# ZhengyiLuo/UHC

Measured on NVIDIA H100. Metric: env_steps_per_s, higher is better.
Workload: dtype f32

## Files before the change

### __graft_entry__.py

```python
import os
import subprocess
import sys

ROOT = os.path.dirname(os.path.abspath(__file__))
if ROOT not in sys.path:
    sys.path.insert(0, ROOT)


def build():
    from uhc_b200 import build as b
    b.build()
    from oracle import oracle as O
    O.build()
    from tests.emu import curriculum_emu, emu, eval_emu, export_emu, group_emu, motion_emu, render_emu, render_mesh_emu, subject_emu, track_emu, video_emu
    emu.build()
    motion_emu.build()
    export_emu.build()
    eval_emu.build()
    curriculum_emu.build()
    track_emu.build()
    group_emu.build()
    render_emu.build()
    render_mesh_emu.build()
    video_emu.build()
    subject_emu.build()
    import uhc_b200
    from uhc_b200 import model
    model.HumanoidModel()


# ... 47 lines not shown
```

### uhc_b200/csrc/env_step.h

```cpp
#pragma once
#include "sim_core.h"
#include "curriculum_core.h"

namespace uhc {

struct CurView {
    const float *pct;
    const int *start;
    const int *meta;
    int max_freq, fit_clip;
    float prec_freq;
};

template <class Real>
struct EngineView {
    Model<Real> model;
    EnvCfg<Real> cfg;
    int num_envs;
    Real *state;
    int *istate;
    const Real *expert;
    const int *clip_adr;
    const Real *clip_shape;
    const int *clip_model;
    const float *clip_cdf;
    const Real *neutral;
    int *ep_log;
    int *ep_start_log;
    int *counters;
    CurView cur;
#if defined(UHC_PHASE_CLOCKS) && !defined(UHC_EMU)
    long long *phase_cyc;
#endif
};

template <class Real>
UHC_DEV bool env_record_valid(const EngineView<Real> &ev, int env) {
    const int *is = ev.istate + (size_t)env * SI_SIZE;
    const int clip = is[SI_CLIP], len = is[SI_LEN];
    return len >= 2 && clip >= 0 && clip < ev.cfg.num_clips;
}
template <class Real, class ObsT>
UHC_DEV void env_step_invalid(const EngineView<Real> &ev, ObsT *obs, ObsT *reward, ObsT *cinfo_out, int *fail_out, int *end_out, ObsT *percent_out) {
    LANES_BEGIN
    if (obs) for (int i = lane; i < ev.cfg.obs_dim; i += 32) obs[i] = (ObsT)0;
    if (cinfo_out && lane < 5) cinfo_out[lane] = (ObsT)0;
    if (lane == 0) {
// ... 273 lines not shown
    LANES_END
    store_state(ev, env, w);
    if (ev.cfg.auto_reset && (fail || end)) {
        int nclip, nstart, nlen;
        const int episode = is[SI_EPISODE] + 1;
        if constexpr (CUR) sample_clip_cur(ev, env, episode, &nclip, &nstart, &nlen);
        else sample_clip(ev, env, episode, &nclip, &nstart, &nlen);
        env_reset_warp<Real, ObsT>(ev, env, w, nclip, nstart, nlen, (const Real *)nullptr, (const Real *)nullptr, obs);
        LANES_BEGIN
        if (lane == 0) is[SI_EPISODE] = episode;
        LANES_END
    }
#if defined(UHC_PHASE_CLOCKS) && !defined(UHC_EMU)
    PCLK(true, w, PC_EPILOGUE);
    if (ev.phase_cyc && (threadIdx.x & 31) == 0) for (int i = 0; i < NPHASE; i++) ev.phase_cyc[(size_t)env * NPHASE + i] += w.pc[i];
#endif
    return fail || end;
}

}
```

### uhc_b200/csrc/sim_core.h

```cpp
#pragma once
#include <math.h>
#include <stdint.h>

#ifndef UHC_EMU
#include <cuda_runtime.h>
#define UHC_DEV __device__ __forceinline__
#define UHC_DEVNI __device__ __noinline__
#define LANES_BEGIN { const int lane = (int)(threadIdx.x & 31);
#define LANES_END } __syncwarp();
#define LANES_END_R }
#define LVAR(T, n) T n
#define LV(n) n
#define LVARA(T, n, K) T n[K]
#define LVA(n) n
#define LV_ARR(n, c) n[c]
#define LV_ALL(n) n
#define UHC_LDG(p) __ldg(p)
__device__ __forceinline__ float uhc_lds(const float *p) { float v; asm("ld.shared.f32 %0, [%1];" : "=f"(v) : "r"((unsigned)__cvta_generic_to_shared(p))); return v; }
__device__ __forceinline__ double uhc_lds(const double *p) { double v; asm("ld.shared.f64 %0, [%1];" : "=d"(v) : "r"((unsigned)__cvta_generic_to_shared(p))); return v; }
__device__ __forceinline__ int uhc_lds(const int *p) { int v; asm("ld.shared.s32 %0, [%1];" : "=r"(v) : "r"((unsigned)__cvta_generic_to_shared(p))); return v; }
#define UHC_LDT(p) uhc_lds(p)
#else
#define UHC_DEV static inline
#define UHC_DEVNI static
// ... 50 lines not shown
    int auto_reset, t_min, t_max, num_clips;
    unsigned long long reset_seed;
    int reactive_v; Real reactive_rate;
    int rfc_mode, vf_dim, act_dim;
    int obs_v, obs_dim;
    int fut_frames, fut_skip;
    int has_shape, obs_block;
    signed char vf_slot[NB];
    int term_body, head_body;
    int reward_mul;
};
constexpr int VF_BODY_DIM = 9, MAX_ACT_DIM = NU + VF_BODY_DIM * NB + 30;

enum { PC_LOAD, PC_PD, PC_KIN, PC_COLLIDE, PC_SMOOTH, PC_CSETUP, PC_NEWTON_ABA, PC_NEWTON_ROWS, PC_SYNC_SUBSTEP, PC_SYNC_PD, PC_SYNC_SMOOTH,
       PC_INTEGRATE, PC_EPILOGUE, NPHASE };

template <class Real>
struct Work {
    alignas(16) Real q[NQ]; Real v[NV + 1], aw[NV + 1], C[NV + 1];
    Real Ib[NB][10];
    alignas(16) Real S[NV + 6][6];
    alignas(16) Real xpos[NB][3]; Real xipos[NB][3], xmat[NB][9];
    Real act[ACT_DIM + 3];
    union {
        struct {
            alignas(16) Real aU[NV + 6][6];
            Real au[NV + 6];
        };
        struct {
            alignas(16) Real xquat[NB][4];
// ... 3 lines not shown
    };
    Real as_[NV + 1], a[NV + 1], g[NV + 1], p[NV + 1], Mp[NV + 1], tau[NV + 1];
    alignas(16) Real Ab[NB][6];
    int cbody[MAXCON]; Real cr[MAXCON][3], cdist[MAXCON], cD[MAXCON], caref[MAXCON][4], cres[MAXCON][4], cjp[MAXCON][4];
    int bcon_adr[NB + 1];
    int ncon, upper_contact;
    int nlim;
    int con_overflow;
    alignas(8) unsigned long long mbar;
    int sync_threads;
    int sync_id;
    alignas(8) Model<Real> mdl;
    alignas(8) EnvCfg<Real> cfg;
#if defined(UHC_PHASE_CLOCKS) && !defined(UHC_EMU)
    long long pc_t, pc[NPHASE];
#endif
};

#if defined(UHC_PHASE_CLOCKS) && !defined(UHC_EMU)
#define PCLK_START(w) do { __syncwarp(); if ((threadIdx.x & 31) == 0) { for (int i_ = 0; i_ < NPHASE; i_++) (w).pc[i_] = 0; (w).pc_t = clock64(); } } while (0)
#define PCLK(on, w, ph) do { if (on) { __syncwarp(); if ((threadIdx.x & 31) == 0) { const long long t_ = clock64(); (w).pc[ph] += t_ - (w).pc_t; (w).pc_t = t_; } } } while (0)
#else
#define PCLK_START(w) do { } while (0)
#define PCLK(on, w, ph) do { (void)sizeof(on); } while (0)
#endif

UHC_DEV float rcp_(float x) {
#if defined(__CUDA_ARCH__)
    float r; asm("rcp.approx.ftz.f32 %0, %1;" : "=f"(r) : "f"(x)); return fmaf(r, fmaf(-x, r, 1.0f), r);
#else
    return 1.0f / x;
#endif
}
UHC_DEV double rcp_(double x) { return 1.0 / x; }
UHC_DEV float rsqrt_(float x) { return 1.0f / sqrtf(x); }
UHC_DEV double rsqrt_(double x) { return 1.0 / sqrt(x); }
UHC_DEV void sincos_(float x, float *s, float *c) {
    const float k = rintf(x * 0.63661977236758134f);
    float r = fmaf(k, -1.5707962512969971f, x);
// ... 93 lines not shown
template <class R> UHC_DEV R warp_sum(R x) {
#pragma unroll 1
    for (int o = 16; o; o >>= 1) x += __shfl_xor_sync(0xffffffffu, x, o);
    return x;
}
template <class R> UHC_DEV R warp_max(R x) { for (int o = 16; o; o >>= 1) { R y = __shfl_xor_sync(0xffffffffu, x, o); x = x > y ? x : y; } return x; }
template <class R> UHC_DEV void warp_argmin(R &x, int &i) {
    for (int o = 16; o; o >>= 1) { R y = __shfl_xor_sync(0xffffffffu, x, o); int j = __shfl_xor_sync(0xffffffffu, i, o); if (y < x || (y == x && j < i)) { x = y; i = j; } }
}
#define WSUM(n) warp_sum(n)
#define WMAX(n) warp_max(n)
#define WARGMIN(x, i, ox, oi) { ox = x; oi = i; warp_argmin(ox, oi); }
#define WBALLOT(n) __ballot_sync(0xffffffffu, (n) != 0)
UHC_DEV int warp_excl_scan(int x, int lane) { int p = x; for (int o = 1; o < 32; o <<= 1) { const int t = __shfl_up_sync(0xffffffffu, p, o); if (lane >= o) p += t; } return p - x; }
#define WEXSCAN(dst, src) { dst = warp_excl_scan(src, (int)(threadIdx.x & 31)); }
template <class R, int K> UHC_DEV void subtree_sum(R (&x)[K], int sub_end, int lane) {
#pragma unroll 1
    for (int o = 1; o < 32; o <<= 1) {
#pragma unroll
        for (int i = 0; i < K; i++) { const R t = __shfl_up_sync(0xffffffffu, x[i], o); if (lane >= o) x[i] += t; }
    }
#pragma unroll
    for (int i = 0; i < K; i++) {
        const R hi = __shfl_sync(0xffffffffu, x[i], sub_end), lo = __shfl_up_sync(0xffffffffu, x[i], 1);
        x[i] = hi - (lane > 0 ? lo : R(0));
    }
}
template <class R, int K> UHC_DEV void ancestor_sum(R (&x)[K], int a1, int a2, int a4, int a8) {
    static_assert(MAXLEVEL + 1 <= 16, "four pointer-jumping rounds cover chains of 16 bodies");
#pragma unroll 1
// ... 10 lines not shown
#pragma unroll
        for (int i = 0; i < K; i++) { const R t = __shfl_up_sync(0xffffffffu, x[i], o); if (lane >= o) x[i] += t; }
    }
}
#define WPREFIX(n, K) prefix_sum<Real, K>(n, (int)(threadIdx.x & 31))
#define WANCESTOR(n, K, tp) ancestor_sum<Real, K>(n, tp.parent, tp.anc2, tp.anc4, tp.anc8)
#else
template <class R> static R emu_sum(const R *x) { R s = 0; for (int i = 0; i < 32; i++) s += x[i]; return s; }
template <class R> static R emu_max(const R *x) { R s = x[0]; for (int i = 1; i < 32; i++) s = x[i] > s ? x[i] : s; return s; }
#define WSUM(n) emu_sum(n)
#define WMAX(n) emu_max(n)
#define WARGMIN(x, i, ox, oi) { ox = x[0]; oi = i[0]; for (int l_ = 1; l_ < 32; l_++) if (x[l_] < ox || (x[l_] == ox && i[l_] < oi)) { ox = x[l_]; oi = i[l_]; } }
static unsigned emu_ballot(const int *x) { unsigned m = 0; for (int i = 0; i < 32; i++) if (x[i]) m |= 1u << i; return m; }
#define WBALLOT(n) emu_ballot(n)
#define WEXSCAN(dst, src) { int run_ = 0; for (int l_ = 0; l_ < 32; l_++) { const int t_ = src[l_]; dst[l_] = run_; run_ += t_; } }
template <class R, int K, class TP> static void emu_subtree(R (*x)[K], const TP *tp) {
    R out[32][K];
    for (int b = 0; b < 32; b++) for (int i = 0; i < K; i++) { R s = 0; for (int c = b; c <= tp[b].sub_end && c < 32; c++) s += x[c][i]; out[b][i] = s; }
    for (int b = 0; b < 32; b++) for (int i = 0; i < K; i++) x[b][i] = out[b][i];
}
template <class R, int K, class TP> static void emu_ancestor(R (*x)[K], const TP *tp) {
    for (int b = 1; b < NB; b++) for (int i = 0; i < K; i++) x[b][i] += x[tp[b].parent][i];
}
#define WSUBTREE(n, K, tp) emu_subtree<Real, K>(n, tp)
#define WPREFIX(n, K) { for (int l_ = 1; l_ < 32; l_++) for (int i_ = 0; i_ < K; i_++) n[l_][i_] += n[l_ - 1][i_]; }
#define WANCESTOR(n, K, tp) emu_ancestor<Real, K>(n, tp)
#endif
UHC_DEV int popc_(unsigned x) { int c = 0; while (x) { x &= x - 1; c++; } return c; }

struct LaneTopo { signed char lane, parent, depth, sub_end, ch0, ch1, ch2, anc2, anc4, anc8; short hnum; int hadr; };
template <class Real>
UHC_DEV LaneTopo lane_topo(const Model<Real> &m, int lane) {
    LaneTopo t; t.lane = lane;
    const int b = lane < NB ? lane : NB - 1;
    t.parent = UHC_LDG(m.parent + b); t.depth = lane < NB ? UHC_LDG(m.depth + b) : 99; t.sub_end = lane < NB ? UHC_LDG(m.body_sub_end + b) : lane;
    const int c0 = UHC_LDG(m.child_adr + b), c1 = UHC_LDG(m.child_adr + b + 1);
    t.ch0 = (lane < NB && c0 < c1) ? UHC_LDG(m.child + c0) : -1;
    t.ch1 = (lane < NB && c0 + 1 < c1) ? UHC_LDG(m.child + c0 + 1) : -1;
    t.ch2 = (lane < NB && c0 + 2 < c1) ? UHC_LDG(m.child + c0 + 2) : -1;
    t.hadr = UHC_LDG(m.hull_adr + b); t.hnum = lane < NB ? UHC_LDG(m.hull_num + b) : 0;
    int a = lane < NB ? b : -1;
    t.anc2 = t.anc4 = t.anc8 = -1;
    for (int k = 1; k <= 8 && a >= 0; ++k) { a = a > 0 ? UHC_LDG(m.parent + a) : -1; if (k == 2) t.anc2 = a; if (k == 4) t.anc4 = a; if (k == 8) t.anc8 = a; }
// ... 243 lines not shown
            paxpy6(x0, S0, a); paxpy6(x1, S1, a); paxpy6(x2, S2, a);
            if (b == 0 && r == 0) {
                x[0] = a[1].y; x[1] = a[2].x; x[2] = a[2].y;
                for (int k = 0; k < 3; k++) x[3 + k] = w.S[3 + k][0] * a[0].x + w.S[3 + k][1] * a[0].y + w.S[3 + k][2] * a[1].x;
            }
        }
        for (int i = 0; i < 3; i++) { LVA(pacc)[2 * i] = a[i].x; LVA(pacc)[2 * i + 1] = a[i].y; }
        if (use_contacts && b >= 0) {
            const P t = r < 2 ? a[0] : (r < 4 ? a[1] : a[2]);
            w.Ab[b][r] = (r & 1) ? t.y : t.x;
        }
        LANES_END
    }
}

template <class Real, class TPT>
UHC_DEV void kin_rne_forward(const Model<Real> &m, Work<Real> &w, const TPT &tp) {
    LVARA(Real, sc, 6);
    LANES_BEGIN
    const int b = lane;
    for (int j = 0; j < 3; ++j) {
        Real sn = 0, cs = 1;
        if (b >= 1 && b < NB) sincos_(w.q[7 + 3 * (b - 1) + j], &sn, &cs);
        LVA(sc)[2 * j] = sn; LVA(sc)[2 * j + 1] = cs;
    }
    LANES_END_R
    for (int lvl = 0; lvl <= MAXLEVEL; ++lvl) {
        LANES_BEGIN
        const int b = lane;
        if (b < NB && TP.depth == lvl) {
            const Real *bf = m.body_f + b * BODYF;
            Real R[9], pos[3]; alignas(16) Real V[6], A[6];
            if (b == 0) {
                Real qn[4] = {w.q[3], w.q[4], w.q[5], w.q[6]};
                Real n = rsqrt_(qn[0] * qn[0] + qn[1] * qn[1] + qn[2] * qn[2] + qn[3] * qn[3]);
                for (int i = 0; i < 4; i++) qn[i] *= n;
                q2mat(qn, R);
                pos[0] = w.q[0]; pos[1] = w.q[1]; pos[2] = w.q[2];
                for (int k = 0; k < 3; k++) {
                    for (int i = 0; i < 6; i++) w.S[k][i] = 0;
                    w.S[k][3 + k] = 1;
                }
                for (int k = 0; k < 3; k++) {
                    w.S[3 + k][0] = R[k]; w.S[3 + k][1] = R[3 + k]; w.S[3 + k][2] = R[6 + k];
                    w.S[3 + k][3] = w.S[3 + k][4] = w.S[3 + k][5] = 0;
                }
                Real wl[3] = {w.v[3], w.v[4], w.v[5]}, ww[3], t[3];
                mv3(R, wl, ww);
                V[0] = ww[0]; V[1] = ww[1]; V[2] = ww[2]; V[3] = w.v[0]; V[4] = w.v[1]; V[5] = w.v[2];
                cross3(ww, V + 3, t);
                A[0] = A[1] = A[2] = 0; A[3] = -t[0]; A[4] = -t[1]; A[5] = -t[2] - m.gravz;
            } else {
                const int p = TP.parent;
                const Real *Rp = w.xmat[p];
                Real off[3] = {UHC_LDG(bf), UHC_LDG(bf + 1), UHC_LDG(bf + 2)};
                mv3(Rp, off, pos);
                for (int i = 0; i < 3; i++) pos[i] += w.xpos[p][i];
                for (int i = 0; i < 9; i++) R[i] = Rp[i];
                for (int i = 0; i < 6; i++) { V[i] = w.Vb[p][i]; A[i] = w.Ab[p][i]; }
                const Real r[3] = {pos[0] - w.q[0], pos[1] - w.q[1], pos[2] - w.q[2]};
#pragma unroll
                for (int j = 0; j < 3; ++j) {
                    const int dof = 6 + 3 * (b - 1) + j, col = 2 - j;
                    Real ax[3] = {R[col], R[3 + col], R[6 + col]}, t[3]; alignas(16) Real Sj[6], Sd[6];
                    cross3(r, ax, t);
                    Sj[0] = ax[0]; Sj[1] = ax[1]; Sj[2] = ax[2]; Sj[3] = t[0]; Sj[4] = t[1]; Sj[5] = t[2];
                    cross3(V, Sj, Sd);
                    cross3(V, Sj + 3, Sd + 3);
                    cross3(V + 3, Sj, t);
                    Sd[3] += t[0]; Sd[4] += t[1]; Sd[5] += t[2];
                    const Real qd = w.v[dof];
                    for (int i = 0; i < 6; i++) w.S[dof][i] = Sj[i];
                    paxpy6(qd, reinterpret_cast<const Pr<Real> *>(Sd), reinterpret_cast<Pr<Real> *>(A));
                    paxpy6(qd, reinterpret_cast<const Pr<Real> *>(Sj), reinterpret_cast<Pr<Real> *>(V));
                    const Real sn = LVA(sc)[2 * j], cs = LVA(sc)[2 * j + 1];
                    const int c1 = (col + 1) % 3, c2 = (col + 2) % 3;
                    for (int i = 0; i < 3; i++) {
                        const Real u = R[3 * i + c1], v2 = R[3 * i + c2];
                        R[3 * i + c1] = cs * u + sn * v2;
                        R[3 * i + c2] = -sn * u + cs * v2;
                    }
                }
            }
            for (int i = 0; i < 3; i++) w.xpos[b][i] = pos[i];
            for (int i = 0; i < 9; i++) w.xmat[b][i] = R[i];
            for (int i = 0; i < 6; i++) { w.Vb[b][i] = V[i]; w.Ab[b][i] = A[i]; }
        }
        LANES_END
    }
    LVARA(Real, IF, 6);
    LANES_BEGIN
    const int b = lane;
    for (int i = 0; i < 6; i++) LVA(IF)[i] = 0;
    if (b < NB) {
        const Real *bf = m.body_f + b * BODYF;
        const Real *R = w.xmat[b], *pos = w.xpos[b], *V = w.Vb[b], *A = w.Ab[b];
        Real cl[3], c[3], I[10], T[9];
        const Real ip[3] = {UHC_LDG(bf + 3), UHC_LDG(bf + 4), UHC_LDG(bf + 5)};
        mv3(R, ip, cl);
        for (int i = 0; i < 3; i++) { w.xipos[b][i] = pos[i] + cl[i]; c[i] = pos[i] + cl[i] - w.q[i]; }
        const Real ms = UHC_LDG(bf + 6);
        const Real i0 = UHC_LDG(bf + 7), i1 = UHC_LDG(bf + 8), i2 = UHC_LDG(bf + 9), i3 = UHC_LDG(bf + 10), i4 = UHC_LDG(bf + 11), i5 = UHC_LDG(bf + 12);
        const Real Il[9] = {i0, i3, i4, i3, i1, i5, i4, i5, i2};
        for (int i = 0; i < 3; i++) for (int j = 0; j < 3; j++) T[3 * i + j] = R[3 * i] * Il[j] + R[3 * i + 1] * Il[3 + j] + R[3 * i + 2] * Il[6 + j];
// ... 2 lines not shown
        I[0] = ms; I[1] = ms * c[0]; I[2] = ms * c[1]; I[3] = ms * c[2];
        for (int e = 0; e < 6; e++) {
            const int i = ii[e], j = jj[e];
            I[4 + e] = T[3 * i] * R[3 * j] + T[3 * i + 1] * R[3 * j + 1] + T[3 * i + 2] * R[3 * j + 2] + ms * ((i == j ? cc : Real(0)) - c[i] * c[j]);
        }
        Real IA[6], IV[6], t[3], t2[3];
        rigid_mul(I, A, IA); rigid_mul(I, V, IV);
        cross3(V, IV, t); cross3(V + 3, IV + 3, t2);
        IA[0] += t[0] + t2[0]; IA[1] += t[1] + t2[1]; IA[2] += t[2] + t2[2];
        cross3(V, IV + 3, t);
        IA[3] += t[0]; IA[4] += t[1]; IA[5] += t[2];
        for (int e = 0; e < 10; e++) w.Ib[b][e] = I[e];
        for (int e = 0; e < 6; e++) LVA(IF)[e] = IA[e];
    }
    LANES_END
    WSUBTREE(IF, 6, tp);
    LANES_BEGIN
    if (lane < NB) for (int e = 0; e < 6; e++) w.Fb[lane][e] = LVA(IF)[e];
    LANES_END
}

template <class Real, class TPT>
UHC_DEVNI void tree_vel(const Model<Real> &m, Work<Real> &w, const Real *x, Real (*X)[6], const TPT &tp) {
    LVARA(Real, V, 6);
    LANES_BEGIN
    const int b = lane;
    Pr<Real> Vp[3] = {pbc(Real(0)), pbc(Real(0)), pbc(Real(0))};
    if (b < NB) {
        const int d0 = b == 0 ? 0 : 6 + 3 * (b - 1), nd = b == 0 ? 6 : 3;
        for (int j = 0; j < nd; ++j) paxpy6(x[d0 + j], as_pairs(w.S[d0 + j]), Vp);
    }
    for (int i = 0; i < 3; i++) { LVA(V)[2 * i] = Vp[i].x; LVA(V)[2 * i + 1] = Vp[i].y; }
    LANES_END_R
    WANCESTOR(V, 6, tp);
// ... 1 lines not shown
    if (lane < NB) for (int i = 0; i < 6; i++) X[lane][i] = LVA(V)[i];
    LANES_END
}
template <class Real>
UHC_DEV void project_force(const Model<Real> &m, Work<Real> &w, const Real (*F)[6], Real *y, Real scale, const Real *add) {
    LANES_BEGIN
#pragma unroll 1
    for (int i = lane; i < NV; i += 32) {
        const int b = i < 6 ? 0 : 1 + (i - 6) / 3;
        y[i] = scale * pdot6(as_pairs(w.S[i]), as_pairs(F[b])) + (add ? add[i] : Real(0));
    }
    LANES_END
}

template <class Real, class TPT>
UHC_DEV void collide(const Model<Real> &m, Work<Real> &w, const TPT &tp) {
    LVAR(int, near); LVAR(int, cnt); LVAR(int, adr0);
    LANES_BEGIN
    int f = 0;
    if (lane < NB) {
        const Real *bf = m.body_f + lane * BODYF; const Real *R = w.xmat[lane];
        const Real cz = w.xpos[lane][2] + R[6] * UHC_LDG(bf + 14) + R[7] * UHC_LDG(bf + 15) + R[8] * UHC_LDG(bf + 16);
        f = !(cz - UHC_LDG(bf + 17) > m.margin);
    }
    LV(near) = f; LV(cnt) = 0;
    LANES_END_R
    unsigned cand_b = WBALLOT(near);
    int ncon = 0, upper = 0;
    while (cand_b) {
        int b = 0; while (!((cand_b >> b) & 1u)) b++;
        cand_b &= cand_b - 1;
        if (ncon + 4 > MAXCON) { w.con_overflow = 1; continue; }
        const Real *R = w.xmat[b];
        const int adr = TP_OF(m, tp, b).hadr, nvt = TP_OF(m, tp, b).hnum;
        LVAR(Real, bz); LVAR(int, bi); LVARA(Real, bv, 3); LVARA(Real, nv, 3);
        LANES_BEGIN
        Real best = Real(1e30); int besti = 1 << 20; Real b0 = 0, b1 = 0, b2 = 0;
        for (int i = lane; i < nvt; i += 32) {
            const Real *vv = m.hull + 3 * (adr + i);
            const Real v0 = UHC_LDG(vv), v1 = UHC_LDG(vv + 1), v2 = UHC_LDG(vv + 2);
            const Real z = w.xpos[b][2] + R[6] * v0 + R[7] * v1 + R[8] * v2;
            if (z < best) { best = z; besti = i; b0 = v0; b1 = v1; b2 = v2; }
        }
        LV(bz) = best; LV(bi) = besti; LVA(bv)[0] = b0; LVA(bv)[1] = b1; LVA(bv)[2] = b2;
        LANES_END_R
        Real minz; int mini;
        WARGMIN(bz, bi, minz, mini);
        if (minz > m.margin) continue;
        const int g = adr + mini, n0 = UHC_LDG(m.nbradr + g), nn = UHC_LDG(m.nbradr + g + 1) - n0;
        LVAR(int, flag);
        LANES_BEGIN
        int f = 0;
        if (lane < nn) {
            const Real *vv = m.hull + 3 * (adr + UHC_LDG(m.nbr + n0 + lane));
            const Real v0 = UHC_LDG(vv), v1 = UHC_LDG(vv + 1), v2 = UHC_LDG(vv + 2);
            const Real z = w.xpos[b][2] + R[6] * v0 + R[7] * v1 + R[8] * v2;
            f = z <= m.margin;
            LVA(nv)[0] = v0; LVA(nv)[1] = v1; LVA(nv)[2] = v2;
        }
        LV(flag) = f;
        LANES_END_R
        const unsigned mask = WBALLOT(flag);
        int nsel = 0; for (unsigned t = mask; t && nsel < 3; t &= t - 1) nsel++;
        const int nc = 1 + nsel;
        LANES_BEGIN
        int below = 0; for (unsigned t = mask & ((1u << lane) - 1u); t; t &= t - 1) below++;
        const bool is_nb = ((mask >> lane) & 1u) && below < 3, is_min = lane == (mini & 31);
        for (int pass = 0; pass < 2; ++pass) {
            if (pass == 0 ? is_min : is_nb) {
                const Real v0 = pass == 0 ? LVA(bv)[0] : LVA(nv)[0], v1 = pass == 0 ? LVA(bv)[1] : LVA(nv)[1], v2 = pass == 0 ? LVA(bv)[2] : LVA(nv)[2];
                const Real px = w.xpos[b][0] + R[0] * v0 + R[1] * v1 + R[2] * v2;
                const Real py = w.xpos[b][1] + R[3] * v0 + R[4] * v1 + R[5] * v2;
                const Real pz = w.xpos[b][2] + R[6] * v0 + R[7] * v1 + R[8] * v2;
                const int c = ncon + (pass == 0 ? 0 : 1 + below);
                w.cbody[c] = b; w.cdist[c] = pz;
                w.cr[c][0] = px - w.q[0]; w.cr[c][1] = py - w.q[1]; w.cr[c][2] = Real(0.5) * pz - w.q[2];
            }
        }
        if (lane == b) LV(cnt) = nc;
        LANES_END
        ncon += nc;
        if (b >= UPPER_BODY0) upper = 1;
    }
    WEXSCAN(LV_ALL(adr0), LV_ALL(cnt));
    LANES_BEGIN
    if (lane <= NB) w.bcon_adr[lane] = LV(adr0);
    LANES_END
    w.ncon = ncon; w.upper_contact = upper;
#ifndef UHC_EMU
    __syncwarp();
#endif
}


template <class Real>
UHC_DEV void constraint_setup(const Model<Real> &m, Work<Real> &w) {
    const Real kk = Real(1) / (m.simp1 * m.simp1 * m.solref0 * m.solref0 * m.solref1 * m.solref1), bb = Real(2) / (m.simp1 * m.solref0);
    LANES_BEGIN
#pragma unroll 1
    for (int c = lane; c < w.ncon; c += 32) {
        const int b = w.cbody[c];
        const Real pos = w.cdist[c] - m.margin;
        Real x = abs_(pos) / m.simp2; if (x > 1) x = 1;
// ... 378 lines not shown
    int phase = with_pd ? PH_PD : PH_SMOOTH, iters = 0;
    bool done = false;
    Real scale = 0, gn2 = 0;
    for (;;) {
        Real *rhs = w.p;
        Real arm_scale = 0;
        if (phase == PH_PD) {
            pd_setup(m, cfg, w, target, it);
            Real sp, sd; pd_gains(cfg, w, it, &sp, &sd);
            arm_scale = sd * m.dt;
        } else if (phase == PH_SMOOTH) {
            Real fapp[6] = {0, 0, 0, 0, 0, 0};
            const bool explicit_rf = with_pd && cfg.rfc_mode == 1 && act_global != nullptr;
            if (explicit_rf) rfc_explicit(m, cfg, w, tp, act_global, w.as_);
            else if (with_pd && cfg.rfc_mode == 0) rfc_implicit(cfg, w, fapp);
            kin_rne_forward(m, w, tp);
            project_force(m, w, w.Fb, w.C, Real(1), (const Real *)nullptr);
            PCLK(cta_sync, w, PC_KIN);
            collide(m, w, tp);
            PCLK(cta_sync, w, PC_COLLIDE);
            LANES_BEGIN
#pragma unroll 1
            for (int i = lane; i < NV; i += 32) {
                Real f = -w.C[i];
                if (explicit_rf) f += w.as_[i];
                else if (i < 6) { const Real fa = i == 0 ? fapp[0] : i == 1 ? fapp[1] : i == 2 ? fapp[2] : i == 3 ? fapp[3] : i == 4 ? fapp[4] : fapp[5]; f += fa; }
                if (i >= 6 && with_pd) f += w.tau[i - 6];
                w.fs[i] = f; w.as_[i] = f;
            }
            LANES_END
            rhs = w.as_;
            limit_setup(m, w);
        } else {
            if (done || iters >= cfg.newton_max_iter || !(gn2 > cfg.newton_tol * cfg.newton_tol * scale * scale)) break;
// ... 259 lines not shown
```

### uhc_b200/csrc/step_kernel.cu

```cuda
#include <cuda_runtime.h>
#include <stdio.h>
#include <stdlib.h>
#include <string.h>
#include <string>
#include <vector>
#include "../../include/uhc_b200.h"
#include "../../include/uhc_eval.h"
#include "../../include/uhc_floor.h"
#include "../../include/uhc_mesh.h"
#include "../../include/uhc_render.h"
#include "../../include/uhc_rollout.h"
#include "../../include/uhc_track.h"
#include "../../include/uhc_video.h"
#include "engine_slots.h"
#include "env_step.h"
#include "errors.h"
#include "motion_core.h"
#include "eval_glue.h"
#include "curriculum_core.h"
#include "track_obs.h"
#include "track_glue.h"
#include "subject_glue.h"

using namespace uhc;
// ... 231 lines not shown
    M.simp0 = (Real)m->solimp[0]; M.simp1 = (Real)m->solimp[1]; M.simp2 = (Real)m->solimp[2]; M.simp3 = (Real)m->solimp[3]; M.simp4 = (Real)m->solimp[4];
    M.gravz = (Real)m->gravz;
    fill_cfg(ev.cfg, cfg);
    ev.num_envs = e->E;
    Real *st; CK(cudaMalloc((void **)&st, (size_t)e->E * ST_SIZE * sizeof(Real))); e->allocs.push_back(st);
    CK(cudaMemset(st, 0, (size_t)e->E * ST_SIZE * sizeof(Real)));
    int *is; CK(cudaMalloc((void **)&is, (size_t)e->E * SI_SIZE * sizeof(int))); e->allocs.push_back(is);
    CK(cudaMemset(is, 0, (size_t)e->E * SI_SIZE * sizeof(int)));
    int *cn; CK(cudaMalloc((void **)&cn, 4 * sizeof(int))); e->allocs.push_back(cn); CK(cudaMemset(cn, 0, 4 * sizeof(int)));
    ev.counters = cn; ev.neutral = nullptr;
    int *el; CK(cudaMalloc((void **)&el, (size_t)e->E * 3 * sizeof(int))); e->allocs.push_back(el); CK(cudaMemset(el, 0xFF, (size_t)e->E * 3 * sizeof(int)));
    ev.ep_log = el; ev.ep_start_log = el + (size_t)2 * e->E;
    ev.cur.pct = nullptr; ev.cur.start = nullptr; ev.cur.meta = nullptr; ev.cur.max_freq = 0; ev.cur.fit_clip = -1; ev.cur.prec_freq = 0.f;
    ev.state = st; ev.istate = is; ev.expert = nullptr; ev.clip_adr = nullptr; ev.clip_shape = nullptr; ev.clip_model = nullptr; ev.clip_cdf = nullptr;
#ifdef UHC_PHASE_CLOCKS
    ev.phase_cyc = nullptr;
#endif
    return 0;
}

constexpr int EPB_F = 16, EPB_D = 2;
template <class Real, int EPB> constexpr size_t step_smem() { return EPB * sizeof(Work<Real>) + 2 * NV * 4 * sizeof(Real) + (MAXLEVEL + 1) * LVL_G * sizeof(int) + 32 * sizeof(LaneTopo); }
static_assert(step_smem<float, EPB_F>() + 1024 + 64 <= 228 * 1024, "k_env_step<float>: the 16 work sets of a block no longer fit one SM");

extern "C" {

const char *uhc_last_error(void) { return uhc_err().c_str(); }
const char *uhc_nn_last_error(void) { return uhc_last_error(); }
const char *uhc_tc_last_error(void) { return uhc_last_error(); }
const char *uhc_ppo_last_error(void) { return uhc_last_error(); }
const char *uhc_rollout_last_error(void) { return uhc_last_error(); }
// ... 323 lines not shown
    else
        k_env_reset<double, EPB_D><<<(n + EPB_D - 1) / EPB_D, 32 * EPB_D, step_smem<double, EPB_D>(), st>>>(e->evd, n, e->d_ids, e->d_ids + n, e->d_ids + 2 * n, e->d_ids + 3 * n, qpos_dev, qvel_dev, obs_dev);
    CK(cudaGetLastError());
    CK(cudaEventRecord(e->ids_done, st));
    e->launches++;
    return 0;
}

#ifdef UHC_PHASE_CLOCKS
int uhc_phase_clocks(UhcEngine *e, long long *buf) {
    if (!e) { uhc_err() = "uhc_phase_clocks: bad argument"; return -2; }
    e->evf.phase_cyc = buf; e->evd.phase_cyc = buf;
    e->view_gen++;
    return NPHASE;
}
#endif

int uhc_env_step(UhcEngine *e, const float *actions_dev, float *obs_dev, float *reward_dev, float *cinfo_dev, int *fail_dev, int *end_dev,
                 float *percent_dev, float *torque_dev, void *stream) {
    if (!e || !actions_dev) { uhc_err() = "uhc_env_step: bad argument"; return -2; }
    if (!e->d_expert) { uhc_err() = "uhc_env_step: no clips loaded"; return -3; }
    CK(cudaSetDevice(e->device));
    cudaStream_t st = (cudaStream_t)stream;
    if (e->d_order) { k_order_envs<<<1, 1024, 0, st>>>(e->precision == 32 ? e->evf.istate : e->evd.istate, e->E, e->d_order); e->launches++; }
    const bool cur = e->cur.M > 0;
    if (e->precision == 32)
        (cur ? k_env_step<float, EPB_F, true> : k_env_step<float, EPB_F>)<<<(e->E + EPB_F - 1) / EPB_F, 32 * EPB_F, step_smem<float, EPB_F>(), st>>>(e->evf, actions_dev, obs_dev, reward_dev, cinfo_dev, fail_dev, end_dev, percent_dev, torque_dev, e->d_order);
    else
        (cur ? k_env_step<double, EPB_D, true> : k_env_step<double, EPB_D>)<<<(e->E + EPB_D - 1) / EPB_D, 32 * EPB_D, step_smem<double, EPB_D>(), st>>>(e->evd, actions_dev, obs_dev, reward_dev, cinfo_dev, fail_dev, end_dev, percent_dev, torque_dev, e->d_order);
    CK(cudaGetLastError());
// ... 439 lines not shown
```

Measured before the change: 1.366 million.

## Parallelize kinematics chain per lane and batch collision narrow phase across bodies

Forward kinematics no longer loops over tree levels with most lanes idle. Each lane now walks its own root-to-body chain, redundantly recomputing its ancestors' transforms, and takes the sin/cos values from the owning lane by shuffle. Collision no longer processes candidate bodies one at a time with a full-warp argmin each. It splits the warp into segments of candidate bodies, does segmented argmin and neighbour-mask reductions, and assigns contact slots with an exclusive scan. It also adds optional sub-phase clock instrumentation, which is compiled out by default, at the cost of redundant arithmetic and more complex shuffle logic.

```diff
diff --git a/__graft_entry__.py b/__graft_entry__.py
--- a/__graft_entry__.py
+++ b/__graft_entry__.py
@@ -12,8 +12,9 @@
     b.build()
     from oracle import oracle as O
     O.build()
-    from tests.emu import curriculum_emu, emu, eval_emu, export_emu, group_emu, motion_emu, render_emu, render_mesh_emu, subject_emu, track_emu, video_emu
+    from tests.emu import curriculum_emu, emu, eval_emu, export_emu, fwd_emu, group_emu, motion_emu, render_emu, render_mesh_emu, subject_emu, track_emu, video_emu
     emu.build()
+    fwd_emu.build()
     motion_emu.build()
     export_emu.build()
     eval_emu.build()
diff --git a/uhc_b200/csrc/env_step.h b/uhc_b200/csrc/env_step.h
--- a/uhc_b200/csrc/env_step.h
+++ b/uhc_b200/csrc/env_step.h
@@ -31,6 +31,7 @@
     CurView cur;
 #if defined(UHC_PHASE_CLOCKS) && !defined(UHC_EMU)
     long long *phase_cyc;
+    long long *phase_sub_cyc;
 #endif
 };
 
@@ -334,6 +335,7 @@
 #if defined(UHC_PHASE_CLOCKS) && !defined(UHC_EMU)
     PCLK(true, w, PC_EPILOGUE);
     if (ev.phase_cyc && (threadIdx.x & 31) == 0) for (int i = 0; i < NPHASE; i++) ev.phase_cyc[(size_t)env * NPHASE + i] += w.pc[i];
+    if (ev.phase_sub_cyc && (threadIdx.x & 31) == 0) for (int i = 0; i < NSUBPHASE; i++) ev.phase_sub_cyc[(size_t)env * NSUBPHASE + i] += w.ps[i];
 #endif
     return fail || end;
 }
diff --git a/uhc_b200/csrc/sim_core.h b/uhc_b200/csrc/sim_core.h
--- a/uhc_b200/csrc/sim_core.h
+++ b/uhc_b200/csrc/sim_core.h
@@ -88,6 +88,7 @@
 
 enum { PC_LOAD, PC_PD, PC_KIN, PC_COLLIDE, PC_SMOOTH, PC_CSETUP, PC_NEWTON_ABA, PC_NEWTON_ROWS, PC_SYNC_SUBSTEP, PC_SYNC_PD, PC_SYNC_SMOOTH,
        PC_INTEGRATE, PC_EPILOGUE, NPHASE };
+enum { PS_KIN_SINCOS, PS_KIN_LEVELS, PS_KIN_INERTIA, PS_KIN_SUBTREE, PS_KIN_PROJECT, PS_COL_BROAD, PS_COL_NARROW, PS_COL_PREFIX, NSUBPHASE };
 
 template <class Real>
 struct Work {
@@ -121,15 +122,19 @@
     alignas(8) EnvCfg<Real> cfg;
 #if defined(UHC_PHASE_CLOCKS) && !defined(UHC_EMU)
     long long pc_t, pc[NPHASE];
+    long long ps_t, ps[NSUBPHASE];
 #endif
 };
 
 #if defined(UHC_PHASE_CLOCKS) && !defined(UHC_EMU)
-#define PCLK_START(w) do { __syncwarp(); if ((threadIdx.x & 31) == 0) { for (int i_ = 0; i_ < NPHASE; i_++) (w).pc[i_] = 0; (w).pc_t = clock64(); } } while (0)
-#define PCLK(on, w, ph) do { if (on) { __syncwarp(); if ((threadIdx.x & 31) == 0) { const long long t_ = clock64(); (w).pc[ph] += t_ - (w).pc_t; (w).pc_t = t_; } } } while (0)
+#define PCLK_START(w) do { __syncwarp(); if ((threadIdx.x & 31) == 0) { for (int i_ = 0; i_ < NPHASE; i_++) (w).pc[i_] = 0; \
+    for (int i_ = 0; i_ < NSUBPHASE; i_++) (w).ps[i_] = 0; (w).pc_t = (w).ps_t = clock64(); } } while (0)
+#define PCLK(on, w, ph) do { if (on) { __syncwarp(); if ((threadIdx.x & 31) == 0) { const long long t_ = clock64(); (w).pc[ph] += t_ - (w).pc_t; (w).pc_t = (w).ps_t = t_; } } } while (0)
+#define PSUB(on, w, sp) do { if (on) { __syncwarp(); if ((threadIdx.x & 31) == 0) { const long long t_ = clock64(); (w).ps[sp] += t_ - (w).ps_t; (w).ps_t = t_; } } } while (0)
 #else
 #define PCLK_START(w) do { } while (0)
 #define PCLK(on, w, ph) do { (void)sizeof(on); } while (0)
+#define PSUB(on, w, sp) do { (void)sizeof(on); } while (0)
 #endif
 
 UHC_DEV float rcp_(float x) {
@@ -253,6 +258,18 @@
 #define WBALLOT(n) __ballot_sync(0xffffffffu, (n) != 0)
 UHC_DEV int warp_excl_scan(int x, int lane) { int p = x; for (int o = 1; o < 32; o <<= 1) { const int t = __shfl_up_sync(0xffffffffu, p, o); if (lane >= o) p += t; } return p - x; }
 #define WEXSCAN(dst, src) { dst = warp_excl_scan(src, (int)(threadIdx.x & 31)); }
+template <class R> UHC_DEV void warp_seg_argmin(R &x, int &i, int G) {
+#pragma unroll 1
+    for (int o = G >> 1; o; o >>= 1) { R y = __shfl_xor_sync(0xffffffffu, x, o); int j = __shfl_xor_sync(0xffffffffu, i, o); if (y < x || (y == x && j < i)) { x = y; i = j; } }
+}
+UHC_DEV unsigned warp_seg_or(unsigned x, int G) {
+#pragma unroll 1
+    for (int o = G >> 1; o; o >>= 1) x |= __shfl_xor_sync(0xffffffffu, x, o);
+    return x;
+}
+#define WSEGARGMIN(x, i, G) warp_seg_argmin(x, i, G)
+#define WSEGOR(x, G) { x = warp_seg_or(x, G); }
+#define WSHFLV(dst, src, SRCL) { const int lane = (int)(threadIdx.x & 31); (void)lane; dst = __shfl_sync(0xffffffffu, src, (SRCL)); }
 template <class R, int K> UHC_DEV void subtree_sum(R (&x)[K], int sub_end, int lane) {
 #pragma unroll 1
     for (int o = 1; o < 32; o <<= 1) {
@@ -293,6 +310,11 @@
 static unsigned emu_ballot(const int *x) { unsigned m = 0; for (int i = 0; i < 32; i++) if (x[i]) m |= 1u << i; return m; }
 #define WBALLOT(n) emu_ballot(n)
 #define WEXSCAN(dst, src) { int run_ = 0; for (int l_ = 0; l_ < 32; l_++) { const int t_ = src[l_]; dst[l_] = run_; run_ += t_; } }
+#define WSEGARGMIN(x, i, G) { for (int g_ = 0; g_ < 32; g_ += (G)) { __typeof__(x[0]) ox_ = x[g_]; int oi_ = i[g_]; \
+    for (int l_ = g_ + 1; l_ < g_ + (G); l_++) if (x[l_] < ox_ || (x[l_] == ox_ && i[l_] < oi_)) { ox_ = x[l_]; oi_ = i[l_]; } \
+    for (int l_ = g_; l_ < g_ + (G); l_++) { x[l_] = ox_; i[l_] = oi_; } } }
+#define WSEGOR(x, G) { for (int g_ = 0; g_ < 32; g_ += (G)) { unsigned o_ = 0; for (int l_ = g_; l_ < g_ + (G); l_++) o_ |= x[l_]; for (int l_ = g_; l_ < g_ + (G); l_++) x[l_] = o_; } }
+#define WSHFLV(dst, src, SRCL) { __typeof__(src[0]) t_[32]; for (int l_ = 0; l_ < 32; l_++) t_[l_] = src[l_]; for (int lane = 0; lane < 32; lane++) dst[lane] = t_[(SRCL)]; }
 template <class R, int K, class TP> static void emu_subtree(R (*x)[K], const TP *tp) {
     R out[32][K];
     for (int b = 0; b < 32; b++) for (int i = 0; i < K; i++) { R s = 0; for (int c = b; c <= tp[b].sub_end && c < 32; c++) s += x[c][i]; out[b][i] = s; }
@@ -305,7 +327,13 @@
 #define WPREFIX(n, K) { for (int l_ = 1; l_ < 32; l_++) for (int i_ = 0; i_ < K; i_++) n[l_][i_] += n[l_ - 1][i_]; }
 #define WANCESTOR(n, K, tp) emu_ancestor<Real, K>(n, tp)
 #endif
-UHC_DEV int popc_(unsigned x) { int c = 0; while (x) { x &= x - 1; c++; } return c; }
+#ifndef UHC_EMU
+UHC_DEV int popc32(unsigned m) { return __popc(m); }
+UHC_DEV int nth_bit(unsigned m, int k) { return (int)__fns(m, 0u, k + 1); }
+#else
+UHC_DEV int popc32(unsigned m) { return __builtin_popcount(m); }
+UHC_DEV int nth_bit(unsigned m, int k) { for (int j = 0; j < k && m; ++j) m &= m - 1; return m ? __builtin_ctz(m) : -1; }
+#endif
 
 struct LaneTopo { signed char lane, parent, depth, sub_end, ch0, ch1, ch2, anc2, anc4, anc8; short hnum; int hadr; };
 template <class Real>
@@ -579,8 +607,66 @@
     }
 }
 
+template <class Real>
+UHC_DEV void kin_root_step(const Model<Real> &m, Work<Real> &w, Real *R, Real *pos, Real *V, Real *A, bool store_S) {
+    Real qn[4] = {w.q[3], w.q[4], w.q[5], w.q[6]};
+    Real n = rsqrt_(qn[0] * qn[0] + qn[1] * qn[1] + qn[2] * qn[2] + qn[3] * qn[3]);
+    for (int i = 0; i < 4; i++) qn[i] *= n;
+    q2mat(qn, R);
+    pos[0] = w.q[0]; pos[1] = w.q[1]; pos[2] = w.q[2];
+    if (store_S) {
+        for (int k = 0; k < 3; k++) {
+            for (int i = 0; i < 6; i++) w.S[k][i] = 0;
+            w.S[k][3 + k] = 1;
+        }
+        for (int k = 0; k < 3; k++) {
+            w.S[3 + k][0] = R[k]; w.S[3 + k][1] = R[3 + k]; w.S[3 + k][2] = R[6 + k];
+            w.S[3 + k][3] = w.S[3 + k][4] = w.S[3 + k][5] = 0;
+        }
+    }
+    Real wl[3] = {w.v[3], w.v[4], w.v[5]}, ww[3], t[3];
+    mv3(R, wl, ww);
+    V[0] = ww[0]; V[1] = ww[1]; V[2] = ww[2]; V[3] = w.v[0]; V[4] = w.v[1]; V[5] = w.v[2];
+    cross3(ww, V + 3, t);
+    A[0] = A[1] = A[2] = 0; A[3] = -t[0]; A[4] = -t[1]; A[5] = -t[2] - m.gravz;
+}
+template <class Real>
+UHC_DEV void kin_hinge_step(Work<Real> &w, int b, const Real *off, const Real *sc, Real *R, Real *pos, Real *V, Real *A, bool store_S) {
+    Real p[3];
+    mv3(R, off, p);
+    for (int i = 0; i < 3; i++) pos[i] += p[i];
+    const Real r[3] = {pos[0] - w.q[0], pos[1] - w.q[1], pos[2] - w.q[2]};
+#pragma unroll
+    for (int j = 0; j < 3; ++j) {
+        const int dof = 6 + 3 * (b - 1) + j, col = 2 - j;
+        Real ax[3] = {R[col], R[3 + col], R[6 + col]}, t[3]; alignas(16) Real Sj[6], Sd[6];
+        cross3(r, ax, t);
+        Sj[0] = ax[0]; Sj[1] = ax[1]; Sj[2] = ax[2]; Sj[3] = t[0]; Sj[4] = t[1]; Sj[5] = t[2];
+        cross3(V, Sj, Sd);
+        cross3(V, Sj + 3, Sd + 3);
+        cross3(V + 3, Sj, t);
+        Sd[3] += t[0]; Sd[4] += t[1]; Sd[5] += t[2];
+        const Real qd = w.v[dof];
+        if (store_S) for (int i = 0; i < 6; i++) w.S[dof][i] = Sj[i];
+        paxpy6(qd, reinterpret_cast<const Pr<Real> *>(Sd), reinterpret_cast<Pr<Real> *>(A));
+        paxpy6(qd, reinterpret_cast<const Pr<Real> *>(Sj), reinterpret_cast<Pr<Real> *>(V));
+        const Real sn = sc[2 * j], cs = sc[2 * j + 1];
+        const int c1 = (col + 1) % 3, c2 = (col + 2) % 3;
+        for (int i = 0; i < 3; i++) {
+            const Real u = R[3 * i + c1], v2 = R[3 * i + c2];
+            R[3 * i + c1] = cs * u + sn * v2;
+            R[3 * i + c2] = -sn * u + cs * v2;
+        }
+    }
+}
+#ifndef UHC_EMU
+#define LGET(n, i, src) __shfl_sync(0xffffffffu, n[i], (src))
+#else
+#define LGET(n, i, src) n[src][i]
+#endif
+
 template <class Real, class TPT>
-UHC_DEV void kin_rne_forward(const Model<Real> &m, Work<Real> &w, const TPT &tp) {
+UHC_DEV void kin_rne_forward(const Model<Real> &m, Work<Real> &w, const TPT &tp, bool clk = false) {
     LVARA(Real, sc, 6);
     LANES_BEGIN
     const int b = lane;
@@ -590,69 +676,36 @@
         LVA(sc)[2 * j] = sn; LVA(sc)[2 * j + 1] = cs;
     }
     LANES_END_R
-    for (int lvl = 0; lvl <= MAXLEVEL; ++lvl) {
-        LANES_BEGIN
-        const int b = lane;
-        if (b < NB && TP.depth == lvl) {
-            const Real *bf = m.body_f + b * BODYF;
-            Real R[9], pos[3]; alignas(16) Real V[6], A[6];
-            if (b == 0) {
-                Real qn[4] = {w.q[3], w.q[4], w.q[5], w.q[6]};
-                Real n = rsqrt_(qn[0] * qn[0] + qn[1] * qn[1] + qn[2] * qn[2] + qn[3] * qn[3]);
-                for (int i = 0; i < 4; i++) qn[i] *= n;
-                q2mat(qn, R);
-                pos[0] = w.q[0]; pos[1] = w.q[1]; pos[2] = w.q[2];
-                for (int k = 0; k < 3; k++) {
-                    for (int i = 0; i < 6; i++) w.S[k][i] = 0;
-                    w.S[k][3 + k] = 1;
-                }
-                for (int k = 0; k < 3; k++) {
-                    w.S[3 + k][0] = R[k]; w.S[3 + k][1] = R[3 + k]; w.S[3 + k][2] = R[6 + k];
-                    w.S[3 + k][3] = w.S[3 + k][4] = w.S[3 + k][5] = 0;
-                }
-                Real wl[3] = {w.v[3], w.v[4], w.v[5]}, ww[3], t[3];
-                mv3(R, wl, ww);
-                V[0] = ww[0]; V[1] = ww[1]; V[2] = ww[2]; V[3] = w.v[0]; V[4] = w.v[1]; V[5] = w.v[2];
-                cross3(ww, V + 3, t);
-                A[0] = A[1] = A[2] = 0; A[3] = -t[0]; A[4] = -t[1]; A[5] = -t[2] - m.gravz;
-            } else {
-                const int p = TP.parent;
-                const Real *Rp = w.xmat[p];
-                Real off[3] = {UHC_LDG(bf), UHC_LDG(bf + 1), UHC_LDG(bf + 2)};
-                mv3(Rp, off, pos);
-                for (int i = 0; i < 3; i++) pos[i] += w.xpos[p][i];
-                for (int i = 0; i < 9; i++) R[i] = Rp[i];
-                for (int i = 0; i < 6; i++) { V[i] = w.Vb[p][i]; A[i] = w.Ab[p][i]; }
-                const Real r[3] = {pos[0] - w.q[0], pos[1] - w.q[1], pos[2] - w.q[2]};
-#pragma unroll
-                for (int j = 0; j < 3; ++j) {
-                    const int dof = 6 + 3 * (b - 1) + j, col = 2 - j;
-                    Real ax[3] = {R[col], R[3 + col], R[6 + col]}, t[3]; alignas(16) Real Sj[6], Sd[6];
-                    cross3(r, ax, t);
-                    Sj[0] = ax[0]; Sj[1] = ax[1]; Sj[2] = ax[2]; Sj[3] = t[0]; Sj[4] = t[1]; Sj[5] = t[2];
-                    cross3(V, Sj, Sd);
-                    cross3(V, Sj + 3, Sd + 3);
-                    cross3(V + 3, Sj, t);
-                    Sd[3] += t[0]; Sd[4] += t[1]; Sd[5] += t[2];
-                    const Real qd = w.v[dof];
-                    for (int i = 0; i < 6; i++) w.S[dof][i] = Sj[i];
-                    paxpy6(qd, reinterpret_cast<const Pr<Real> *>(Sd), reinterpret_cast<Pr<Real> *>(A));
-                    paxpy6(qd, reinterpret_cast<const Pr<Real> *>(Sj), reinterpret_cast<Pr<Real> *>(V));
-                    const Real sn = LVA(sc)[2 * j], cs = LVA(sc)[2 * j + 1];
-                    const int c1 = (col + 1) % 3, c2 = (col + 2) % 3;
-                    for (int i = 0; i < 3; i++) {
-                        const Real u = R[3 * i + c1], v2 = R[3 * i + c2];
-                        R[3 * i + c1] = cs * u + sn * v2;
-                        R[3 * i + c2] = -sn * u + cs * v2;
-                    }
-                }
-            }
-            for (int i = 0; i < 3; i++) w.xpos[b][i] = pos[i];
-            for (int i = 0; i < 9; i++) w.xmat[b][i] = R[i];
-            for (int i = 0; i < 6; i++) { w.Vb[b][i] = V[i]; w.Ab[b][i] = A[i]; }
-        }
-        LANES_END
-    }
+    PSUB(clk, w, PS_KIN_SINCOS);
+    LANES_BEGIN
+    const int b = lane, depth = b < NB ? (int)TP.depth : 0;
+    Real R[9], pos[3]; alignas(16) Real V[6], A[6];
+    kin_root_step(m, w, R, pos, V, A, b == 0);
+    int a = 0;
+#pragma unroll 1
+    for (int d = 1; d <= MAXLEVEL; ++d) {
+        const LaneTopo &ta = TP_OF(m, tp, a);
+        int c = ta.ch0;
+        if (ta.ch1 >= 0 && ta.ch1 <= b) c = ta.ch1;
+        if (ta.ch2 >= 0 && ta.ch2 <= b) c = ta.ch2;
+        const bool act = d <= depth;
+        if (!act) c = 0;
+        Real s[6];
+        for (int i = 0; i < 6; i++) s[i] = LGET(sc, i, c);
+        if (act) {
+            const Real *bf = m.body_f + c * BODYF;
+            const Real off[3] = {UHC_LDG(bf), UHC_LDG(bf + 1), UHC_LDG(bf + 2)};
+            kin_hinge_step(w, c, off, s, R, pos, V, A, c == b);
+            a = c;
+        }
+    }
+    if (b < NB) {
+        for (int i = 0; i < 3; i++) w.xpos[b][i] = pos[i];
+        for (int i = 0; i < 9; i++) w.xmat[b][i] = R[i];
+        for (int i = 0; i < 6; i++) { w.Vb[b][i] = V[i]; w.Ab[b][i] = A[i]; }
+    }
+    LANES_END
+    PSUB(clk, w, PS_KIN_LEVELS);
     LVARA(Real, IF, 6);
     LANES_BEGIN
     const int b = lane;
@@ -685,10 +738,12 @@
         for (int e = 0; e < 6; e++) LVA(IF)[e] = IA[e];
     }
     LANES_END
+    PSUB(clk, w, PS_KIN_INERTIA);
     WSUBTREE(IF, 6, tp);
     LANES_BEGIN
     if (lane < NB) for (int e = 0; e < 6; e++) w.Fb[lane][e] = LVA(IF)[e];
     LANES_END
+    PSUB(clk, w, PS_KIN_SUBTREE);
 }
 
 template <class Real, class TPT>
@@ -720,7 +775,7 @@
 }
 
 template <class Real, class TPT>
-UHC_DEV void collide(const Model<Real> &m, Work<Real> &w, const TPT &tp) {
+UHC_DEV void collide(const Model<Real> &m, Work<Real> &w, const TPT &tp, bool clk = false) {
     LVAR(int, near); LVAR(int, cnt); LVAR(int, adr0);
     LANES_BEGIN
     int f = 0;
@@ -729,70 +784,97 @@
         const Real cz = w.xpos[lane][2] + R[6] * UHC_LDG(bf + 14) + R[7] * UHC_LDG(bf + 15) + R[8] * UHC_LDG(bf + 16);
         f = !(cz - UHC_LDG(bf + 17) > m.margin);
     }
-    LV(near) = f; LV(cnt) = 0;
+    LV(near) = f;
     LANES_END_R
     unsigned cand_b = WBALLOT(near);
-    int ncon = 0, upper = 0;
-    while (cand_b) {
-        int b = 0; while (!((cand_b >> b) & 1u)) b++;
-        cand_b &= cand_b - 1;
-        if (ncon + 4 > MAXCON) { w.con_overflow = 1; continue; }
+    PSUB(clk, w, PS_COL_BROAD);
+    const int ncand = popc32(cand_b);
+    int lg = 5; while ((ncand << lg) > 32) lg--;
+    const int G = 1 << lg;
+    LVAR(int, cb); LVAR(Real, bz); LVAR(int, bi); LVAR(unsigned, nmask); LVAR(int, nck); LVAR(int, exk); LVAR(int, acc); LVAR(int, ovf); LVAR(int, up);
+    LANES_BEGIN
+    const int k = lane >> lg, sub = lane & (G - 1);
+    Real best = Real(1e30); int besti = 1 << 20, b = -1;
+    if (k < ncand) {
+        b = nth_bit(cand_b, k);
         const Real *R = w.xmat[b];
         const int adr = TP_OF(m, tp, b).hadr, nvt = TP_OF(m, tp, b).hnum;
-        LVAR(Real, bz); LVAR(int, bi); LVARA(Real, bv, 3); LVARA(Real, nv, 3);
-        LANES_BEGIN
-        Real best = Real(1e30); int besti = 1 << 20; Real b0 = 0, b1 = 0, b2 = 0;
-        for (int i = lane; i < nvt; i += 32) {
+#pragma unroll 1
+        for (int i = sub; i < nvt; i += G) {
             const Real *vv = m.hull + 3 * (adr + i);
             const Real v0 = UHC_LDG(vv), v1 = UHC_LDG(vv + 1), v2 = UHC_LDG(vv + 2);
             const Real z = w.xpos[b][2] + R[6] * v0 + R[7] * v1 + R[8] * v2;
-            if (z < best) { best = z; besti = i; b0 = v0; b1 = v1; b2 = v2; }
-        }
-        LV(bz) = best; LV(bi) = besti; LVA(bv)[0] = b0; LVA(bv)[1] = b1; LVA(bv)[2] = b2;
-        LANES_END_R
-        Real minz; int mini;
-        WARGMIN(bz, bi, minz, mini);
-        if (minz > m.margin) continue;
-        const int g = adr + mini, n0 = UHC_LDG(m.nbradr + g), nn = UHC_LDG(m.nbradr + g + 1) - n0;
-        LVAR(int, flag);
-        LANES_BEGIN
-        int f = 0;
-        if (lane < nn) {
-            const Real *vv = m.hull + 3 * (adr + UHC_LDG(m.nbr + n0 + lane));
+            if (z < best) { best = z; besti = i; }
+        }
+    }
+    LV(cb) = b; LV(bz) = best; LV(bi) = besti;
+    LANES_END_R
+    WSEGARGMIN(LV_ALL(bz), LV_ALL(bi), G);
+    LANES_BEGIN
+    const int k = lane >> lg, sub = lane & (G - 1), b = LV(cb);
+    unsigned f = 0;
+    if (k < ncand && !(LV(bz) > m.margin)) {
+        const Real *R = w.xmat[b];
+        const int adr = TP_OF(m, tp, b).hadr, g = adr + LV(bi), n0 = UHC_LDG(m.nbradr + g), nn = min_(UHC_LDG(m.nbradr + g + 1) - n0, 32);
+#pragma unroll 1
+        for (int j = sub; j < nn; j += G) {
+            const Real *vv = m.hull + 3 * (adr + UHC_LDG(m.nbr + n0 + j));
             const Real v0 = UHC_LDG(vv), v1 = UHC_LDG(vv + 1), v2 = UHC_LDG(vv + 2);
             const Real z = w.xpos[b][2] + R[6] * v0 + R[7] * v1 + R[8] * v2;
-            f = z <= m.margin;
-            LVA(nv)[0] = v0; LVA(nv)[1] = v1; LVA(nv)[2] = v2;
-        }
-        LV(flag) = f;
-        LANES_END_R
-        const unsigned mask = WBALLOT(flag);
-        int nsel = 0; for (unsigned t = mask; t && nsel < 3; t &= t - 1) nsel++;
-        const int nc = 1 + nsel;
-        LANES_BEGIN
-        int below = 0; for (unsigned t = mask & ((1u << lane) - 1u); t; t &= t - 1) below++;
-        const bool is_nb = ((mask >> lane) & 1u) && below < 3, is_min = lane == (mini & 31);
-        for (int pass = 0; pass < 2; ++pass) {
-            if (pass == 0 ? is_min : is_nb) {
-                const Real v0 = pass == 0 ? LVA(bv)[0] : LVA(nv)[0], v1 = pass == 0 ? LVA(bv)[1] : LVA(nv)[1], v2 = pass == 0 ? LVA(bv)[2] : LVA(nv)[2];
-                const Real px = w.xpos[b][0] + R[0] * v0 + R[1] * v1 + R[2] * v2;
-                const Real py = w.xpos[b][1] + R[3] * v0 + R[4] * v1 + R[5] * v2;
-                const Real pz = w.xpos[b][2] + R[6] * v0 + R[7] * v1 + R[8] * v2;
-                const int c = ncon + (pass == 0 ? 0 : 1 + below);
-                w.cbody[c] = b; w.cdist[c] = pz;
-                w.cr[c][0] = px - w.q[0]; w.cr[c][1] = py - w.q[1]; w.cr[c][2] = Real(0.5) * pz - w.q[2];
-            }
-        }
-        if (lane == b) LV(cnt) = nc;
-        LANES_END
-        ncon += nc;
-        if (b >= UPPER_BODY0) upper = 1;
-    }
+            if (z <= m.margin) f |= 1u << j;
+        }
+    }
+    LV(nmask) = f;
+    LANES_END_R
+    WSEGOR(LV_ALL(nmask), G);
+    LANES_BEGIN
+    int nc = 0;
+    if ((lane >> lg) < ncand && !(LV(bz) > m.margin)) { const int nsel = popc32(LV(nmask)); nc = 1 + (nsel < 3 ? nsel : 3); }
+    LV(nck) = nc;
+    LANES_END_R
+    WSHFLV(LV_ALL(exk), LV_ALL(nck), (lane < ncand ? lane << lg : 31));
+    LANES_BEGIN
+    if (lane >= ncand) LV(exk) = 0;
+    LV(acc) = LV(exk);
+    LANES_END_R
+    WEXSCAN(LV_ALL(exk), LV_ALL(acc));
+    LANES_BEGIN
+    const bool ok = LV(exk) + 4 <= MAXCON;
+    LV(ovf) = lane < ncand && !ok;
+    LV(up) = lane < ncand && ok && LV(acc) > 0 && nth_bit(cand_b, lane) >= UPPER_BODY0;
+    if (!ok) LV(acc) = 0;
+    LANES_END_R
+    if (WBALLOT(ovf)) w.con_overflow = 1;
+    const int upper = WBALLOT(up) != 0;
+    WSHFLV(LV_ALL(cnt), LV_ALL(acc), (((cand_b >> lane) & 1u) ? popc32(cand_b & ((1u << lane) - 1u)) : 31));
+    WSHFLV(LV_ALL(nck), LV_ALL(acc), lane >> lg);
+    WSHFLV(LV_ALL(exk), LV_ALL(exk), lane >> lg);
+    LANES_BEGIN
+    const int nc = LV(nck), b = LV(cb);
+    if (nc > 0) {
+        const Real *R = w.xmat[b];
+        const int adr = TP_OF(m, tp, b).hadr, g = adr + LV(bi);
+#pragma unroll 1
+        for (int c = lane & (G - 1); c < nc; c += G) {
+            const int vi = c == 0 ? g : adr + UHC_LDG(m.nbr + UHC_LDG(m.nbradr + g) + nth_bit(LV(nmask), c - 1));
+            const Real *vv = m.hull + 3 * vi;
+            const Real v0 = UHC_LDG(vv), v1 = UHC_LDG(vv + 1), v2 = UHC_LDG(vv + 2);
+            const Real px = w.xpos[b][0] + R[0] * v0 + R[1] * v1 + R[2] * v2;
+            const Real py = w.xpos[b][1] + R[3] * v0 + R[4] * v1 + R[5] * v2;
+            const Real pz = w.xpos[b][2] + R[6] * v0 + R[7] * v1 + R[8] * v2;
+            const int slot = LV(exk) + c;
+            w.cbody[slot] = b; w.cdist[slot] = pz;
+            w.cr[slot][0] = px - w.q[0]; w.cr[slot][1] = py - w.q[1]; w.cr[slot][2] = Real(0.5) * pz - w.q[2];
+        }
+    }
+    LANES_END
+    PSUB(clk, w, PS_COL_NARROW);
     WEXSCAN(LV_ALL(adr0), LV_ALL(cnt));
     LANES_BEGIN
     if (lane <= NB) w.bcon_adr[lane] = LV(adr0);
-    LANES_END
-    w.ncon = ncon; w.upper_contact = upper;
+    if (lane == NB) w.ncon = LV(adr0);
+    LANES_END
+    w.upper_contact = upper;
 #ifndef UHC_EMU
     __syncwarp();
 #endif
@@ -1201,10 +1283,12 @@
             const bool explicit_rf = with_pd && cfg.rfc_mode == 1 && act_global != nullptr;
             if (explicit_rf) rfc_explicit(m, cfg, w, tp, act_global, w.as_);
             else if (with_pd && cfg.rfc_mode == 0) rfc_implicit(cfg, w, fapp);
-            kin_rne_forward(m, w, tp);
+            kin_rne_forward(m, w, tp, cta_sync);
             project_force(m, w, w.Fb, w.C, Real(1), (const Real *)nullptr);
+            PSUB(cta_sync, w, PS_KIN_PROJECT);
             PCLK(cta_sync, w, PC_KIN);
-            collide(m, w, tp);
+            collide(m, w, tp, cta_sync);
+            PSUB(cta_sync, w, PS_COL_PREFIX);
             PCLK(cta_sync, w, PC_COLLIDE);
             LANES_BEGIN
 #pragma unroll 1
diff --git a/uhc_b200/csrc/step_kernel.cu b/uhc_b200/csrc/step_kernel.cu
--- a/uhc_b200/csrc/step_kernel.cu
+++ b/uhc_b200/csrc/step_kernel.cu
@@ -269,7 +269,7 @@
     ev.cur.pct = nullptr; ev.cur.start = nullptr; ev.cur.meta = nullptr; ev.cur.max_freq = 0; ev.cur.fit_clip = -1; ev.cur.prec_freq = 0.f;
     ev.state = st; ev.istate = is; ev.expert = nullptr; ev.clip_adr = nullptr; ev.clip_shape = nullptr; ev.clip_model = nullptr; ev.clip_cdf = nullptr;
 #ifdef UHC_PHASE_CLOCKS
-    ev.phase_cyc = nullptr;
+    ev.phase_cyc = nullptr; ev.phase_sub_cyc = nullptr;
 #endif
     return 0;
 }
@@ -623,6 +623,12 @@
     e->view_gen++;
     return NPHASE;
 }
+int uhc_phase_subclocks(UhcEngine *e, long long *buf) {
+    if (!e) { uhc_err() = "uhc_phase_subclocks: bad argument"; return -2; }
+    e->evf.phase_sub_cyc = buf; e->evd.phase_sub_cyc = buf;
+    e->view_gen++;
+    return NSUBPHASE;
+}
 #endif
 
 int uhc_env_step(UhcEngine *e, const float *actions_dev, float *obs_dev, float *reward_dev, float *cinfo_dev, int *fail_dev, int *end_dev,
```

Result: faster. 1.407 million (median of 6 runs) (+3.0%).
